# Zilong-Li/BaseVarC

Measured on AMD Instinct MI355X. Metric: sites/sec at N=1e6 samples; achieved HBM GB/s vs roofline, higher is better.
Workload: dtype f64

## Files before the change

basevarc_amd/csrc/bgzf_deflate_kernel.hip:

```cpp
#include "bvc_device.h"
#include "bvc_internal.h"
#include "crc32_device.h"

namespace bvc {

namespace {

constexpr int kBdThreads = 1024;
constexpr int kBdRound = 256;
constexpr int kBdLanes = kBdThreads / kBdRound;
constexpr int kBdWays = 16, kBdHashBits = 11, kBdHash = 1 << kBdHashBits;
constexpr int kBdWaysPerLane = kBdWays / kBdLanes;
constexpr uint32_t kBdIn = BVC_BGZF_BLOCK_INPUT;
constexpr uint32_t kBdSlot = 65536;
constexpr uint32_t kBdMinMatch = 4, kBdMaxMatch = 258, kBdMaxDist = 32768;
constexpr uint32_t kBdMatchBit = 0x80000000u;
constexpr int kBdInWords = kBdSlot / 4 + 4;
constexpr int kBdTabWords = kBdWays / 2 * kBdHash;
constexpr int kBdBitWords = kBdHash;
static_assert(kBdTabWords * 4 >= (int)kBdIn && kBdBitWords * 32 >= (int)kBdIn && kBdHash == 2048, "what takes the tables' place fits");
static_assert((kBdInWords + kBdTabWords + 2 * kBdBitWords + 32) * 4 <= 160 * 1024, "one workgroup's LDS");
static_assert(kBdIn % 64 == 0 && kBdIn / 64 <= kBdThreads, "64 positions a thread in pass C");
static_assert(kBdWays == 16 && kBdRound == 256, "the packing of the table's and the round's cells");

struct BlockDesc { int64_t src; uint32_t len; uint32_t pad; };

__device__ __forceinline__ uint32_t ld32(const uint32_t *w, uint32_t a)
{
    const uint32_t i = a >> 2;
    const uint64_t v = (uint64_t)w[i] | ((uint64_t)w[i + 1] << 32);
    return (uint32_t)(v >> ((a & 3u) * 8u));
}

__device__ __forceinline__ uint32_t hash_of(uint32_t four) { return (four * 2654435761u) >> (32 - kBdHashBits); }

__device__ __forceinline__ uint32_t rev_bits(uint32_t x, uint32_t n) { return __brev(x) >> (32u - n); }

__device__ __forceinline__ uint32_t literal_bits(uint32_t b, uint32_t &bits)
{
    if (b < 144u) { bits = rev_bits(0x30u + b, 8u); return 8u; }
    bits = rev_bits(0x190u + (b - 144u), 9u);
    return 9u;
}
__device__ __forceinline__ uint32_t match_bits(uint32_t len, uint32_t dist, uint32_t &bits)
{
    const uint32_t l = len - 3u;
    uint32_t sym, le = 0u, lx = 0u;
    if (len == 258u) sym = 285u;
    else if (l < 8u) sym = 257u + l;
    else { le = (31u - (uint32_t)__clz((int)l)) - 2u; sym = 261u + 4u * le + ((l >> le) & 3u); lx = l & ((1u << le) - 1u); }
    uint32_t n;
    if (sym <= 279u) { bits = rev_bits(sym - 256u, 7u); n = 7u; } else { bits = rev_bits(0xC0u + (sym - 280u), 8u); n = 8u; }
    bits |= lx << n; n += le;
    const uint32_t d = dist - 1u;
    uint32_t ds, de = 0u, dx = 0u;
    if (d < 4u) ds = d;
    else { de = (31u - (uint32_t)__clz((int)d)) - 1u; ds = 2u * de + 2u + ((d >> de) & 1u); dx = d & ((1u << de) - 1u); }
    bits |= rev_bits(ds, 5u) << n; n += 5u;
    bits |= dx << n; n += de;
    return n;
}

}

__global__ __launch_bounds__(256) void bgzf_plan_kernel(
    int64_t n_pieces, const int64_t *__restrict__ piece_off, const int64_t *__restrict__ piece_len, const int64_t *__restrict__ first_block,
    int64_t n_blocks, BlockDesc *__restrict__ desc)
{
    for (int64_t b = (int64_t)blockIdx.x * 256 + threadIdx.x; b < n_blocks; b += (int64_t)gridDim.x * 256) {
        int64_t lo = 0, hi = n_pieces - 1;
        while (lo < hi) {
            const int64_t mid = (lo + hi + 1) >> 1;
            if (first_block[mid] <= b) lo = mid; else hi = mid - 1;
        }
        const int64_t at = (b - first_block[lo]) * (int64_t)kBdIn, left = piece_len[lo] - at;
        BlockDesc d;
        d.src = piece_off[lo] + at;
        d.len = left <= 0 ? 0u : (left < (int64_t)kBdIn ? (uint32_t)left : kBdIn);
        d.pad = 0u;
        desc[b] = d;
    }
}

__global__ __launch_bounds__(kBdThreads) void bgzf_deflate_kernel(
    const uint8_t *__restrict__ data, const BlockDesc *__restrict__ desc, int64_t n_blocks, uint8_t *__restrict__ staging,
    uint32_t *__restrict__ bsize, uint32_t *__restrict__ match_rows)
{
    BVC_POISON_LDS();
    __shared__ __attribute__((aligned(16))) uint32_t s_in[kBdInWords];
    __shared__ __attribute__((aligned(16))) uint32_t s_tab[kBdTabWords];
    __shared__ uint32_t s_first[kBdBitWords];
    __shared__ uint32_t s_path[kBdBitWords];
    __shared__ uint32_t s_scan[32];
    const uint32_t tid = threadIdx.x, lane = tid & (kWave - 1), wave = tid >> 6;
    uint32_t *const match = match_rows + (size_t)blockIdx.x * kBdIn;
    uint32_t *const s_out = s_in;
    uint8_t *const s_sym = reinterpret_cast<uint8_t *>(s_tab);
    uint32_t *const s_ism = s_first;

    for (int64_t blk = blockIdx.x; blk < n_blocks; blk += gridDim.x) {
        const uint32_t n = desc[blk].len < kBdIn ? desc[blk].len : kBdIn;
        uint8_t *const slot = staging + (size_t)blk * kBdSlot;
        if (n == 0u) {
            if (tid == 0u) bsize[blk] = 0u;
            continue;
        }
        const uint8_t *__restrict__ src = data + desc[blk].src;
        {
            const uint32_t head = (uint32_t)(reinterpret_cast<uintptr_t>(src) & 3u);
            const uint32_t *__restrict__ g = reinterpret_cast<const uint32_t *>(src - head);
            for (uint32_t w = tid; w < (uint32_t)kBdInWords; w += kBdThreads) {
                uint32_t v = 0u;
                if (4u * w < n) {
                    const uint32_t lo = g[w];
                    const uint32_t hi = head != 0u && 4u * (w + 1u) < n + head ? g[w + 1u] : 0u;
                    v = (uint32_t)((((uint64_t)hi << 32) | lo) >> (8u * head));
                    const uint32_t left = n - 4u * w;
                    if (left < 4u) v &= (1u << (8u * left)) - 1u;
                }
                s_in[w] = v;
            }
        }
        for (uint32_t w = tid; w < (uint32_t)kBdTabWords; w += kBdThreads) s_tab[w] = 0u;
        for (uint32_t w = tid; w < (uint32_t)kBdBitWords; w += kBdThreads) s_first[w] = 0u;
        __syncthreads();

        const uint32_t sub = tid & (kBdLanes - 1), slotpos = tid / kBdLanes;
        const uint32_t rounds = (n + kBdRound - 1) / kBdRound;
        uint32_t prev_h = 0u, prev_p = 0u;
        bool prev_ok = false;
        for (uint32_t r = 0; r < rounds; ++r) {
            const uint32_t p = r * kBdRound + slotpos;
            const bool ok = p + 4u <= n;
            const uint32_t four = ok ? ld32(s_in, p) : 0u;
            const uint32_t h = hash_of(four);
            if (sub == 0u) {
                if (prev_ok && BVC_LDS_OK(0x901, prev_h, kBdHash)) {
                    const uint32_t way = (r - 1u) & (kBdWays - 1u);
                    uint32_t *const cell = &s_tab[(way & 7u) * kBdHash + prev_h];
                    const uint32_t cur = *cell;
                    atomicMax(cell, way >> 3 ? (cur & 0xFFFFu) | ((prev_p + 1u) << 16) : (cur & 0xFFFF0000u) | (prev_p + 1u));
                }
                if (ok && BVC_LDS_OK(0x902, h, kBdHash)) atomicMax(&s_first[h], ((r + 1u) << 8) | (255u - slotpos));
            }
            __syncthreads();
            uint32_t best = 0u, best_d = 0u;
            if (ok) {
                const uint32_t mx = n - p < kBdMaxMatch ? n - p : kBdMaxMatch;
                auto consider = [&](uint32_t q) {
                    const uint32_t d = p - q;
                    if (d > kBdMaxDist || best == mx) return;
                    if (best >= kBdMinMatch && ld32(s_in, q + best - 3u) != ld32(s_in, p + best - 3u)) return;
                    uint32_t l = 0u;
                    while (l < mx) {
                        const uint32_t x = ld32(s_in, q + l) ^ ld32(s_in, p + l);
                        if (x != 0u) { l += (uint32_t)__builtin_ctz(x) >> 3; break; }
                        l += 4u;
                    }
                    l = l < mx ? l : mx;
                    if (l > best) { best = l; best_d = d; }
                };
#pragma unroll
                for (uint32_t k = 0; k < (uint32_t)kBdWaysPerLane; ++k) {
                    const uint32_t way = sub * kBdWaysPerLane + k;
                    const uint32_t cell = s_tab[(way & 7u) * kBdHash + h];
                    const uint32_t q1 = way >> 3 ? cell >> 16 : cell & 0xFFFFu;
                    if (q1 != 0u && q1 - 1u < p && BVC_LDS_OK(0x903, q1 - 1u, kBdIn)) consider(q1 - 1u);
                }
                if (sub == 0u) {
                    const uint32_t f = s_first[h];
                    const uint32_t q = r * kBdRound + 255u - (f & 255u);
                    if ((f >> 8) == r + 1u && q < p && BVC_LDS_OK(0x904, q, kBdIn)) consider(q);
                }
            }
            uint32_t key = best >= kBdMinMatch ? (best << 16) | (kBdMaxDist - best_d) : 0u;
#pragma unroll
            for (int d = 1; d < kBdLanes; d <<= 1) {
                const uint32_t o = (uint32_t)__shfl_xor((int)key, d);
                key = o > key ? o : key;
            }
            if (sub == 0u && p < n)
                match[p] = key != 0u ? kBdMatchBit | (((key >> 16) - 3u) << 16) | (kBdMaxDist - (key & 0xFFFFu) - 1u) : 0u;
            prev_h = h; prev_p = p; prev_ok = ok;
            __syncthreads();
        }
        __threadfence();
        __syncthreads();

        for (uint32_t g = tid; g < kBdIn / 32u; g += kBdThreads) {
            uint32_t ism = 0u;
#pragma unroll
            for (uint32_t j = 0; j < 8u; ++j) {
                const uint32_t p0 = 32u * g + 4u * j;
                uint32_t packed = 0u;
                if (p0 < n) {
                    const uint4 m4 = *reinterpret_cast<const uint4 *>(match + p0);
                    const uint32_t m[4] = {m4.x, m4.y, m4.z, m4.w};
                    const uint32_t lit = s_in[p0 >> 2];
#pragma unroll
                    for (uint32_t k = 0; k < 4u; ++k) {
                        const bool is = p0 + k < n && (m[k] & kBdMatchBit) != 0u;
                        ism |= is ? 1u << (4u * j + k) : 0u;
                        packed |= (is ? (m[k] >> 16) & 0xFFu : (lit >> (8u * k)) & 0xFFu) << (8u * k);
                    }
                }
                s_tab[8u * g + j] = packed;
            }
            s_ism[g] = ism;
            s_path[g] = 0u;
        }
        __syncthreads();
        if (tid == 0u) {
            uint32_t p = 0u;
            while (p < n) {
                const uint32_t w = p >> 5, b = p & 31u;
                const uint32_t m = s_ism[w] >> b;
                if (m == 0u) { s_path[w] |= ~0u << b; p = (w + 1u) << 5; continue; }
                const uint32_t k = (uint32_t)__builtin_ctz(m);
                s_path[w] |= (((1u << k) - 1u) | (1u << k)) << b;
                p += k;
                p += (uint32_t)s_sym[p] + 3u;
            }
        }
        __syncthreads();

        uint32_t my_bits = 0u;
        uint64_t mask = 0u;
        const uint32_t base = 64u * tid;
        if (base < n) {
            mask = (uint64_t)s_path[2u * tid] | ((uint64_t)s_path[2u * tid + 1u] << 32);
            if (n - base < 64u) mask &= (1ull << (n - base)) - 1ull;
            const uint64_t ism = (uint64_t)s_ism[2u * tid] | ((uint64_t)s_ism[2u * tid + 1u] << 32);
            for (uint64_t left = mask; left != 0u; left &= left - 1u) {
                const uint32_t p = base + (uint32_t)__builtin_ctzll(left);
                uint32_t bits;
                my_bits += (ism >> (p - base)) & 1u ? match_bits((uint32_t)s_sym[p] + 3u, (match[p] & 0x7FFFu) + 1u, bits)
                                                   : literal_bits(s_sym[p], bits);
            }
        }
        uint32_t incl = my_bits;
#pragma unroll
        for (int d = 1; d < kWave; d <<= 1) {
            const uint32_t o = (uint32_t)__shfl_up((int)incl, d);
            incl += lane >= (uint32_t)d ? o : 0u;
        }
        if (lane == kWave - 1) s_scan[wave] = incl;
        __syncthreads();
        uint32_t before = 0u, all = 0u;
#pragma unroll
        for (uint32_t v = 0; v < kBdThreads / kWave; ++v) {
            const uint32_t s = s_scan[v];
            before += v < wave ? s : 0u;
            all += s;
        }
        const uint32_t total_bits = 3u + all + 7u;
        const uint32_t coded = (total_bits + 7u) >> 3;
        const bool stored = coded > n + 5u;
        const uint32_t csize = stored ? n + 5u : coded;
        const uint32_t out_words = (csize + 3u) >> 2;
        if (!stored) {
            for (uint32_t w = tid; w < out_words; w += kBdThreads) s_out[w] = 0u;
            __syncthreads();
            if (base < n) {
                uint32_t at = 3u + before + incl - my_bits;
                uint32_t word = at >> 5, fill = at & 31u;
                uint64_t acc = tid == 0u ? 3u : 0u;
                const uint64_t ism = (uint64_t)s_ism[2u * tid] | ((uint64_t)s_ism[2u * tid + 1u] << 32);
                for (uint64_t left = mask; left != 0u; left &= left - 1u) {
                    const uint32_t p = base + (uint32_t)__builtin_ctzll(left);
                    uint32_t bits;
                    const uint32_t nb = (ism >> (p - base)) & 1u ? match_bits((uint32_t)s_sym[p] + 3u, (match[p] & 0x7FFFu) + 1u, bits)
                                                                : literal_bits(s_sym[p], bits);
                    acc |= (uint64_t)bits << fill;
                    fill += nb;
                    if (fill >= 32u) {
                        if (BVC_LDS_OK(0x905, word, out_words)) atomicOr(&s_out[word], (uint32_t)acc);
                        acc >>= 32; fill -= 32u; ++word;
                    }
                }
                if (acc != 0u && BVC_LDS_OK(0x906, word, out_words)) atomicOr(&s_out[word], (uint32_t)acc);
            }
            __syncthreads();
        }
        const uint32_t bs = csize + 26u;
        {
            auto byte_at = [&](uint32_t x) -> uint32_t {
                if (x < 18u) {
                    const uint32_t word = x < 4u ? 0x04088b1fu : x < 8u ? 0u : x < 12u ? 0x0006ff00u : x < 16u ? 0x00024342u : (bs - 1u) & 0xFFFFu;
                    return (word >> (8u * (x & 3u))) & 0xFFu;
                }
                const uint32_t i = x - 18u;
                if (i < csize) {
                    if (!stored) return (s_out[i >> 2] >> (8u * (i & 3u))) & 0xFFu;
                    if (i < 5u) return ((i < 4u ? 0x01u | (n << 8) | ((~n & 0xFFu) << 24) : (~n >> 8) & 0xFFu) >> (8u * (i & 3u))) & 0xFFu;
                    return (s_in[(i - 5u) >> 2] >> (8u * ((i - 5u) & 3u))) & 0xFFu;
                }
                const uint32_t t = i - csize;
                return t >= 4u && t < 8u ? (n >> (8u * (t - 4u))) & 0xFFu : 0u;
            };
            uint32_t *const slot32 = reinterpret_cast<uint32_t *>(slot);
            const uint32_t first = stored ? 23u : 18u;
            for (uint32_t k = tid; 4u * k < bs; k += kBdThreads) {
                uint32_t v;
                if (4u * k >= first && 4u * k + 4u <= 18u + csize) v = ld32(stored ? s_in : s_out, 4u * k - first);
                else v = byte_at(4u * k) | (byte_at(4u * k + 1u) << 8) | (byte_at(4u * k + 2u) << 16) | (byte_at(4u * k + 3u) << 24);
                slot32[k] = v;
            }
        }
        if (tid == 0u) bsize[blk] = bs;
        __syncthreads();
    }
}

__global__ __launch_bounds__(kWave) void bgzf_crc_kernel(const uint8_t *__restrict__ data16, uint32_t shift, const BlockDesc *__restrict__ desc,
                                                         int64_t n_blocks, const uint32_t *__restrict__ bsize, uint8_t *__restrict__ staging)
{
    BVC_POISON_LDS();
    __shared__ uint32_t tab[256];
    const int lane = threadIdx.x;
    crc_table_fill(tab, lane);
    for (int64_t blk = blockIdx.x; blk < n_blocks; blk += gridDim.x) {
        const uint32_t n = desc[blk].len < kBdIn ? desc[blk].len : kBdIn;
        if (n == 0u) continue;
        const uint32_t crc = crc32_wave(data16, (uint64_t)desc[blk].src + shift, n, tab, lane);
        const uint32_t bs = bsize[blk] <= kBdSlot ? bsize[blk] : kBdSlot;
        if (lane < 4 && bs >= 26u) staging[(size_t)blk * kBdSlot + bs - 8u + (uint32_t)lane] = (uint8_t)(crc >> (8 * lane));
    }
}

__global__ __launch_bounds__(1024) void bgzf_scan_kernel(int64_t n_blocks, const uint32_t *__restrict__ bsize, int64_t *__restrict__ block_off,
                                                         int64_t n_pieces, const int64_t *__restrict__ first_block, int64_t *__restrict__ comp_off)
{
    BVC_POISON_LDS();
    __shared__ int64_t s_sz[1024];
    const int tid = threadIdx.x;
    int64_t base = 0;
    for (int64_t b0 = 0; b0 < n_blocks; b0 += 1024) {
        const int64_t b = b0 + tid;
        const int64_t sz = b < n_blocks ? (int64_t)bsize[b] : 0;
        s_sz[tid] = sz;
        __syncthreads();
        for (int d = 1; d < 1024; d <<= 1) {
            const int64_t v = tid >= d ? s_sz[tid - d] : 0;
            __syncthreads();
            s_sz[tid] += v;
            __syncthreads();
        }
        if (b < n_blocks) block_off[b] = base + s_sz[tid] - sz;
        const int64_t tot = s_sz[1023];
        __syncthreads();
        base += tot;
    }
    if (tid == 0) block_off[n_blocks] = base;
    __threadfence();
    __syncthreads();
    for (int64_t i = tid; i <= n_pieces; i += 1024) comp_off[i] = block_off[first_block[i]];
}

__global__ __launch_bounds__(256) void bgzf_pack_kernel(int64_t n_blocks, const uint32_t *__restrict__ bsize, const int64_t *__restrict__ block_off,
                                                        const uint8_t *__restrict__ staging, uint8_t *__restrict__ comp, int64_t comp_cap)
{
    if (block_off[n_blocks] > comp_cap) return;
    for (int64_t blk = blockIdx.x; blk < n_blocks; blk += gridDim.x) {
        const uint32_t bs = bsize[blk] <= kBdSlot - 8u ? bsize[blk] : kBdSlot - 8u;
        const uint32_t *__restrict__ from = reinterpret_cast<const uint32_t *>(staging + (size_t)blk * kBdSlot);
        uint8_t *__restrict__ to = comp + block_off[blk];
        const uint32_t lead = (uint32_t)(-reinterpret_cast<uintptr_t>(to) & 3u);
        const uint32_t head = lead < bs ? lead : bs, words = (bs - head) >> 2, tail = head + 4u * words;
        if (threadIdx.x < head) to[threadIdx.x] = (uint8_t)(from[0] >> (8u * threadIdx.x));
        uint32_t *__restrict__ to32 = reinterpret_cast<uint32_t *>(to + head);
        for (uint32_t j = threadIdx.x; j < words; j += 256) {
            const uint32_t at = head + 4u * j;
            const uint64_t v = (uint64_t)from[at >> 2] | ((uint64_t)from[(at >> 2) + 1u] << 32);
            to32[j] = (uint32_t)(v >> (8u * (at & 3u)));
        }
        if (threadIdx.x < bs - tail) {
            const uint32_t at = tail + threadIdx.x;
            to[at] = (uint8_t)(from[at >> 2] >> (8u * (at & 3u)));
        }
    }
}

size_t bgzf_deflate_scratch_bytes(int64_t n_pieces, int64_t n_blocks)
{
    Layout L;
    (void)bgzf_deflate_scratch(nullptr, n_pieces, n_blocks, &L);
    return L.at;
}

BgzfDeflateScratch bgzf_deflate_scratch(void *buf, int64_t n_pieces, int64_t n_blocks, Layout *sized)
{
    Layout L{reinterpret_cast<uintptr_t>(buf)};
    const size_t nb = (size_t)n_blocks, grid = nb < (size_t)kBgzfDeflateGrid ? nb : (size_t)kBgzfDeflateGrid;
    BgzfDeflateScratch s;
    s.first_block = L.take<int64_t>((size_t)n_pieces + 1);
    s.block_off = L.take<int64_t>(nb + 1);
    s.desc = L.take<char>(nb * sizeof(BlockDesc));
    s.bsize = L.take<uint32_t>(nb);
    s.match_rows = L.take<uint32_t>(grid * kBdIn);
    s.staging = L.take<uint8_t>(nb * kBdSlot);
    if (sized) *sized = L;
    return s;
}

hipError_t launch_bgzf_deflate(hipStream_t stream, int64_t n_pieces, const uint8_t *data, const int64_t *piece_off, const int64_t *piece_len,
                               int64_t n_blocks, const BgzfDeflateScratch &s, uint8_t *comp, int64_t comp_cap, int64_t *comp_off)
{
    BlockDesc *const desc = reinterpret_cast<BlockDesc *>(s.desc);
    if (n_blocks > 0) {
        const unsigned grid = (unsigned)(n_blocks < kBgzfDeflateGrid ? n_blocks : kBgzfDeflateGrid);
        hipLaunchKernelGGL(bgzf_plan_kernel, dim3((unsigned)((n_blocks + 255) / 256 < 1024 ? (n_blocks + 255) / 256 : 1024)), dim3(256), 0, stream,
                           n_pieces, piece_off, piece_len, s.first_block, n_blocks, desc);
        hipLaunchKernelGGL(bgzf_deflate_kernel, dim3(grid), dim3(kBdThreads), 0, stream, data, desc, n_blocks, s.staging, s.bsize, s.match_rows);
        const uintptr_t a = reinterpret_cast<uintptr_t>(data);
        hipLaunchKernelGGL(bgzf_crc_kernel, dim3((unsigned)(n_blocks < 65536 ? n_blocks : 65536)), dim3(kWave), 0, stream,
                           reinterpret_cast<const uint8_t *>(a & ~(uintptr_t)15), (uint32_t)(a & 15u), desc, n_blocks, s.bsize, s.staging);
    }
    hipLaunchKernelGGL(bgzf_scan_kernel, dim3(1), dim3(1024), 0, stream, n_blocks, s.bsize, s.block_off, n_pieces, s.first_block, comp_off);
    if (n_blocks > 0)
        hipLaunchKernelGGL(bgzf_pack_kernel, dim3((unsigned)(n_blocks < 2048 ? n_blocks : 2048)), dim3(256), 0, stream, n_blocks, s.bsize,
                           s.block_off, s.staging, comp, comp_cap);
    return hipGetLastError();
}

#ifdef BVC_CHECK_LDS
BVC_DEFINE_DEBUG_READER(debug_read_bgzf_deflate)
#endif

}
```

Measured before the change: 3.377 million.

## Parallelize deflate match search within quads and chunk the greedy parse path

Match finding now screens all candidates with a 16-byte compare, then extends surviving candidates cooperatively across the four lanes of a quad using DPP min/max reductions and 8-byte loads, instead of each lane walking its candidates serially. The match-row store is deferred past the next barrier. The single-thread greedy parse over the whole block becomes a per-64-position chunk exit table computed in parallel, so one thread only hops between chunks and each thread then rebuilds its own path mask. ld32 uses alignbyte, and the stored-block fallback reloads the input. This aims to cut divergent serial match loops and the serial parse, at the cost of more code complexity and extra LDS traffic.

New measurement: 3.375 million (median of 2 runs). Within noise of the previous version (-0.1%).

```diff
diff --git a/basevarc_amd/csrc/bgzf_deflate_kernel.hip b/basevarc_amd/csrc/bgzf_deflate_kernel.hip
--- a/basevarc_amd/csrc/bgzf_deflate_kernel.hip
+++ b/basevarc_amd/csrc/bgzf_deflate_kernel.hip
@@ -15,21 +15,89 @@
 constexpr uint32_t kBdSlot = 65536;
 constexpr uint32_t kBdMinMatch = 4, kBdMaxMatch = 258, kBdMaxDist = 32768;
 constexpr uint32_t kBdMatchBit = 0x80000000u;
+constexpr uint32_t kBdScreen = 16;
+constexpr uint32_t kBdChunk = 64;
+constexpr uint32_t kBdNone = 0xFFFFFFFFu;
 constexpr int kBdInWords = kBdSlot / 4 + 4;
 constexpr int kBdTabWords = kBdWays / 2 * kBdHash;
 constexpr int kBdBitWords = kBdHash;
 static_assert(kBdTabWords * 4 >= (int)kBdIn && kBdBitWords * 32 >= (int)kBdIn && kBdHash == 2048, "what takes the tables' place fits");
 static_assert((kBdInWords + kBdTabWords + 2 * kBdBitWords + 32) * 4 <= 160 * 1024, "one workgroup's LDS");
-static_assert(kBdIn % 64 == 0 && kBdIn / 64 <= kBdThreads, "64 positions a thread in pass C");
+static_assert(kBdChunk == 64 && kBdIn % kBdChunk == 0 && kBdIn / kBdChunk <= kBdThreads, "64 positions a thread in passes B and C: one 64-bit mask");
+static_assert(kBdLanes == 4 && kBdWaysPerLane == 4 && kBdScreen == 16, "a quad a position in pass A, four words screened");
+static_assert(kBdChunk - 1 + kBdMaxMatch - kBdChunk < 512, "a chunk's exit, relative to its end, in nine bits");
 static_assert(kBdWays == 16 && kBdRound == 256, "the packing of the table's and the round's cells");
 
 struct BlockDesc { int64_t src; uint32_t len; uint32_t pad; };
 
+#ifdef BVC_DIAG_KNOBS
+#define BVC_BD_STOP_PARAM , int dbg_stop
+#define BVC_BD_STOP_ARG , bgzf_dbg_stop()
+#define BVC_BD_STOP(k)                                                                                            \
+    if (dbg_stop == (k)) {                                                                                        \
+        if (tid == 0u) bsize[blk] = 0u;                                                                           \
+        __syncthreads();                                                                                          \
+        continue;                                                                                                 \
+    }
+#else
+#define BVC_BD_STOP_PARAM
+#define BVC_BD_STOP_ARG
+#define BVC_BD_STOP(k)
+#endif
+
 __device__ __forceinline__ uint32_t ld32(const uint32_t *w, uint32_t a)
 {
     const uint32_t i = a >> 2;
-    const uint64_t v = (uint64_t)w[i] | ((uint64_t)w[i + 1] << 32);
-    return (uint32_t)(v >> ((a & 3u) * 8u));
+    return __builtin_amdgcn_alignbyte(w[i + 1], w[i], a & 3u);
+}
+__device__ __forceinline__ uint64_t ld64_aligned(const uint32_t *w, uint32_t a)
+{
+    const uint32_t i = a >> 2;
+    return (uint64_t)w[i] | ((uint64_t)w[i + 1] << 32);
+}
+__device__ __forceinline__ uint64_t ld64(const uint32_t *w, uint32_t a)
+{
+    const uint32_t i = a >> 2, by = a & 3u;
+    const uint32_t w0 = w[i], w1 = w[i + 1], w2 = w[i + 2];
+    return (uint64_t)__builtin_amdgcn_alignbyte(w1, w0, by) | ((uint64_t)__builtin_amdgcn_alignbyte(w2, w1, by) << 32);
+}
+__device__ __forceinline__ void ld128(const uint32_t *w, uint32_t a, uint32_t (&b)[4])
+{
+    const uint32_t i = a >> 2, by = a & 3u;
+    const uint32_t w0 = w[i], w1 = w[i + 1], w2 = w[i + 2], w3 = w[i + 3], w4 = w[i + 4];
+    b[0] = __builtin_amdgcn_alignbyte(w1, w0, by);
+    b[1] = __builtin_amdgcn_alignbyte(w2, w1, by);
+    b[2] = __builtin_amdgcn_alignbyte(w3, w2, by);
+    b[3] = __builtin_amdgcn_alignbyte(w4, w3, by);
+}
+__device__ __forceinline__ uint32_t first_difference(uint32_t x0, uint32_t x1, uint32_t x2, uint32_t x3)
+{
+    const uint32_t lo = x0 != 0u ? x0 : x1, hi = x2 != 0u ? x2 : x3;
+    const uint32_t at_lo = x0 != 0u ? 0u : 4u, at_hi = x2 != 0u ? 8u : 12u;
+    const bool in_lo = (x0 | x1) != 0u;
+    const uint32_t x = in_lo ? lo : hi, at = in_lo ? at_lo : at_hi;
+    return x != 0u ? at + ((uint32_t)__builtin_ctz(x) >> 3) : 16u;
+}
+
+template <int XOR>
+__device__ __forceinline__ uint32_t quad_xor(uint32_t v)
+{
+    static_assert(XOR == 1 || XOR == 2, "inside a quad");
+    return (uint32_t)__builtin_amdgcn_update_dpp(0, (int)v, XOR == 1 ? 0xB1 : 0x4E, 0xF, 0xF, false);
+}
+__device__ __forceinline__ uint32_t quad_max(uint32_t v)
+{
+    const uint32_t a = quad_xor<1>(v);
+    v = a > v ? a : v;
+    const uint32_t b = quad_xor<2>(v);
+    return b > v ? b : v;
+}
+__device__ __forceinline__ uint32_t quad_min(uint32_t v)
+{
+    const uint32_t a = quad_xor<1>(v);
+    v = a < v ? a : v;
+    const uint32_t b = quad_xor<2>(v);
+    return b < v ? b : v;
 }
 
 __device__ __forceinline__ uint32_t hash_of(uint32_t four) { return (four * 2654435761u) >> (32 - kBdHashBits); }
@@ -84,7 +152,7 @@
 
 __global__ __launch_bounds__(kBdThreads) void bgzf_deflate_kernel(
     const uint8_t *__restrict__ data, const BlockDesc *__restrict__ desc, int64_t n_blocks, uint8_t *__restrict__ staging,
-    uint32_t *__restrict__ bsize, uint32_t *__restrict__ match_rows)
+    uint32_t *__restrict__ bsize, uint32_t *__restrict__ match_rows BVC_BD_STOP_PARAM)
 {
     BVC_POISON_LDS();
     __shared__ __attribute__((aligned(16))) uint32_t s_in[kBdInWords];
@@ -96,6 +164,7 @@
     uint32_t *const match = match_rows + (size_t)blockIdx.x * kBdIn;
     uint32_t *const s_out = s_in;
     uint8_t *const s_sym = reinterpret_cast<uint8_t *>(s_tab);
+    uint8_t *const s_exit = reinterpret_cast<uint8_t *>(s_in);
     uint32_t *const s_ism = s_first;
 
     for (int64_t blk = blockIdx.x; blk < n_blocks; blk += gridDim.x) {
@@ -106,7 +175,7 @@
             continue;
         }
         const uint8_t *__restrict__ src = data + desc[blk].src;
-        {
+        auto load_input = [&]() {
             const uint32_t head = (uint32_t)(reinterpret_cast<uintptr_t>(src) & 3u);
             const uint32_t *__restrict__ g = reinterpret_cast<const uint32_t *>(src - head);
             for (uint32_t w = tid; w < (uint32_t)kBdInWords; w += kBdThreads) {
@@ -120,20 +189,23 @@
                 }
                 s_in[w] = v;
             }
-        }
+        };
+        load_input();
         for (uint32_t w = tid; w < (uint32_t)kBdTabWords; w += kBdThreads) s_tab[w] = 0u;
         for (uint32_t w = tid; w < (uint32_t)kBdBitWords; w += kBdThreads) s_first[w] = 0u;
         __syncthreads();
+        BVC_BD_STOP(1)
 
         const uint32_t sub = tid & (kBdLanes - 1), slotpos = tid / kBdLanes;
         const uint32_t rounds = (n + kBdRound - 1) / kBdRound;
-        uint32_t prev_h = 0u, prev_p = 0u;
-        bool prev_ok = false;
+        uint32_t prev_h = 0u, prev_p = 0u, prev_m = 0u;
+        bool prev_ok = false, prev_store = false;
         for (uint32_t r = 0; r < rounds; ++r) {
             const uint32_t p = r * kBdRound + slotpos;
             const bool ok = p + 4u <= n;
-            const uint32_t four = ok ? ld32(s_in, p) : 0u;
-            const uint32_t h = hash_of(four);
+            uint32_t at_p[4] = {0u, 0u, 0u, 0u};
+            if (ok) ld128(s_in, p, at_p);
+            const uint32_t h = hash_of(at_p[0]);
             if (sub == 0u) {
                 if (prev_ok && BVC_LDS_OK(0x901, prev_h, kBdHash)) {
                     const uint32_t way = (r - 1u) & (kBdWays - 1u);
@@ -144,48 +216,75 @@
                 if (ok && BVC_LDS_OK(0x902, h, kBdHash)) atomicMax(&s_first[h], ((r + 1u) << 8) | (255u - slotpos));
             }
             __syncthreads();
-            uint32_t best = 0u, best_d = 0u;
+            if (prev_store) match[prev_p] = prev_m;
+            uint32_t key = 0u;
             if (ok) {
                 const uint32_t mx = n - p < kBdMaxMatch ? n - p : kBdMaxMatch;
-                auto consider = [&](uint32_t q) {
-                    const uint32_t d = p - q;
-                    if (d > kBdMaxDist || best == mx) return;
-                    if (best >= kBdMinMatch && ld32(s_in, q + best - 3u) != ld32(s_in, p + best - 3u)) return;
-                    uint32_t l = 0u;
-                    while (l < mx) {
-                        const uint32_t x = ld32(s_in, q + l) ^ ld32(s_in, p + l);
-                        if (x != 0u) { l += (uint32_t)__builtin_ctz(x) >> 3; break; }
-                        l += 4u;
-                    }
-                    l = l < mx ? l : mx;
-                    if (l > best) { best = l; best_d = d; }
-                };
+                uint32_t cand[kBdWaysPerLane + 1];
+                bool has[kBdWaysPerLane + 1];
 #pragma unroll
                 for (uint32_t k = 0; k < (uint32_t)kBdWaysPerLane; ++k) {
                     const uint32_t way = sub * kBdWaysPerLane + k;
                     const uint32_t cell = s_tab[(way & 7u) * kBdHash + h];
                     const uint32_t q1 = way >> 3 ? cell >> 16 : cell & 0xFFFFu;
-                    if (q1 != 0u && q1 - 1u < p && BVC_LDS_OK(0x903, q1 - 1u, kBdIn)) consider(q1 - 1u);
-                }
-                if (sub == 0u) {
+                    has[k] = q1 != 0u && q1 - 1u < p && p - (q1 - 1u) <= kBdMaxDist && BVC_LDS_OK(0x903, q1 - 1u, kBdIn);
+                    cand[k] = has[k] ? q1 - 1u : p;
+                }
+                {
                     const uint32_t f = s_first[h];
                     const uint32_t q = r * kBdRound + 255u - (f & 255u);
-                    if ((f >> 8) == r + 1u && q < p && BVC_LDS_OK(0x904, q, kBdIn)) consider(q);
-                }
-            }
-            uint32_t key = best >= kBdMinMatch ? (best << 16) | (kBdMaxDist - best_d) : 0u;
-#pragma unroll
-            for (int d = 1; d < kBdLanes; d <<= 1) {
-                const uint32_t o = (uint32_t)__shfl_xor((int)key, d);
-                key = o > key ? o : key;
-            }
-            if (sub == 0u && p < n)
-                match[p] = key != 0u ? kBdMatchBit | (((key >> 16) - 3u) << 16) | (kBdMaxDist - (key & 0xFFFFu) - 1u) : 0u;
+                    has[kBdWaysPerLane] = sub == 0u && (f >> 8) == r + 1u && q < p && BVC_LDS_OK(0x904, q, kBdIn);
+                    cand[kBdWaysPerLane] = has[kBdWaysPerLane] ? q : p;
+                }
+                uint32_t surv[kBdWaysPerLane + 1];
+#pragma unroll
+                for (uint32_t k = 0; k <= (uint32_t)kBdWaysPerLane; ++k) {
+                    uint32_t at_q[4];
+                    ld128(s_in, cand[k], at_q);
+                    uint32_t m = first_difference(at_q[0] ^ at_p[0], at_q[1] ^ at_p[1], at_q[2] ^ at_p[2], at_q[3] ^ at_p[3]);
+                    m = m < mx ? m : mx;
+                    const bool more = m == kBdScreen && mx > kBdScreen;
+                    surv[k] = has[k] && more ? cand[k] + 1u : 0u;
+                    const uint32_t mk = has[k] && !more && m >= kBdMinMatch ? (m << 16) | (kBdMaxDist - (p - cand[k])) : 0u;
+                    key = mk > key ? mk : key;
+                }
+                uint32_t best = 0u, best_d = 0u;
+                for (;;) {
+                    uint32_t mine = surv[0];
+#pragma unroll
+                    for (uint32_t k = 1; k <= (uint32_t)kBdWaysPerLane; ++k) mine = surv[k] > mine ? surv[k] : mine;
+                    const uint32_t top = quad_max(mine);
+                    if (top == 0u || best == mx) break;
+#pragma unroll
+                    for (uint32_t k = 0; k <= (uint32_t)kBdWaysPerLane; ++k) surv[k] = surv[k] == top ? 0u : surv[k];
+                    const uint32_t q = top - 1u;
+                    if (best != 0u && ld32(s_in, q + best - 3u) != ld32(s_in, p + best - 3u)) continue;
+                    const uint32_t o0 = kBdScreen - (p & 3u);
+                    uint32_t l = mx;
+                    for (uint32_t o = o0; o < mx; o += 8u * kBdLanes) {
+                        const uint32_t mo = o + 8u * sub;
+                        uint32_t miss = kBdNone;
+                        if (mo < mx) {
+                            const uint64_t x = ld64(s_in, q + mo) ^ ld64_aligned(s_in, p + mo);
+                            if (x != 0u) miss = mo + ((uint32_t)__builtin_ctzll(x) >> 3);
+                        }
+                        miss = quad_min(miss);
+                        if (miss != kBdNone) { l = miss < mx ? miss : mx; break; }
+                    }
+                    if (l > best) { best = l; best_d = p - q; }
+                }
+                if (best != 0u) key = (best << 16) | (kBdMaxDist - best_d);
+                key = quad_max(key);
+            }
+            prev_store = sub == 0u && p < n;
+            prev_m = key != 0u ? kBdMatchBit | (((key >> 16) - 3u) << 16) | (kBdMaxDist - (key & 0xFFFFu) - 1u) : 0u;
             prev_h = h; prev_p = p; prev_ok = ok;
             __syncthreads();
         }
+        if (prev_store) match[prev_p] = prev_m;
         __threadfence();
         __syncthreads();
+        BVC_BD_STOP(2)
 
         for (uint32_t g = tid; g < kBdIn / 32u; g += kBdThreads) {
             uint32_t ism = 0u;
@@ -207,30 +306,57 @@
                 s_tab[8u * g + j] = packed;
             }
             s_ism[g] = ism;
-            s_path[g] = 0u;
+        }
+        __syncthreads();
+        const uint32_t base = kBdChunk * tid;
+        uint64_t ism = 0u, mask = 0u;
+        if (base < n) {
+            ism = (uint64_t)s_ism[2u * tid] | ((uint64_t)s_ism[2u * tid + 1u] << 32);
+            uint64_t ninth = 0u;
+            uint32_t leave = 0u;
+            for (int i = (int)kBdChunk - 1; i >= 0; --i) {
+                if ((ism >> i) & 1u) {
+                    const uint32_t to = (uint32_t)i + (uint32_t)s_sym[base + (uint32_t)i] + 3u;
+                    leave = to >= kBdChunk ? to - kBdChunk
+                                          : (uint32_t)s_exit[base + to] | ((uint32_t)(ninth >> to) & 1u) << 8;
+                }
+                s_exit[base + (uint32_t)i] = (uint8_t)leave;
+                ninth |= (uint64_t)(leave >> 8) << i;
+            }
+            s_path[2u * tid] = (uint32_t)ninth;
+            s_path[2u * tid + 1u] = (uint32_t)(ninth >> 32);
         }
         __syncthreads();
         if (tid == 0u) {
             uint32_t p = 0u;
-            while (p < n) {
-                const uint32_t w = p >> 5, b = p & 31u;
-                const uint32_t m = s_ism[w] >> b;
-                if (m == 0u) { s_path[w] |= ~0u << b; p = (w + 1u) << 5; continue; }
-                const uint32_t k = (uint32_t)__builtin_ctz(m);
-                s_path[w] |= (((1u << k) - 1u) | (1u << k)) << b;
-                p += k;
-                p += (uint32_t)s_sym[p] + 3u;
-            }
-        }
-        __syncthreads();
+            for (uint32_t c = 0; kBdChunk * c < n; ++c) {
+                uint32_t enters = kBdNone;
+                const uint32_t end = kBdChunk * (c + 1u);
+                if (p < end && p < n && BVC_LDS_OK(0x907, p, kBdIn)) {
+                    enters = p - kBdChunk * c;
+                    const uint32_t nine = (s_path[2u * c + (enters >> 5)] >> (enters & 31u)) & 1u;
+                    p = end + (uint32_t)s_exit[p] + (nine << 8);
+                }
+                s_path[2u * c] = enters;
+            }
+        }
+        __syncthreads();
+        if (base < n) {
+            uint32_t at = s_path[2u * tid];
+            while (at < kBdChunk) {
+                const uint64_t m = ism >> at;
+                if (m == 0u) { mask |= ~0ull << at; break; }
+                const uint32_t k = (uint32_t)__builtin_ctzll(m);
+                mask |= ((2ull << k) - 1ull) << at;
+                at += k;
+                at += (uint32_t)s_sym[base + at] + 3u;
+            }
+            if (n - base < kBdChunk) mask &= (1ull << (n - base)) - 1ull;
+        }
+        BVC_BD_STOP(3)
 
         uint32_t my_bits = 0u;
-        uint64_t mask = 0u;
-        const uint32_t base = 64u * tid;
         if (base < n) {
-            mask = (uint64_t)s_path[2u * tid] | ((uint64_t)s_path[2u * tid + 1u] << 32);
-            if (n - base < 64u) mask &= (1ull << (n - base)) - 1ull;
-            const uint64_t ism = (uint64_t)s_ism[2u * tid] | ((uint64_t)s_ism[2u * tid + 1u] << 32);
             for (uint64_t left = mask; left != 0u; left &= left - 1u) {
                 const uint32_t p = base + (uint32_t)__builtin_ctzll(left);
                 uint32_t bits;
@@ -265,7 +391,6 @@
                 uint32_t at = 3u + before + incl - my_bits;
                 uint32_t word = at >> 5, fill = at & 31u;
                 uint64_t acc = tid == 0u ? 3u : 0u;
-                const uint64_t ism = (uint64_t)s_ism[2u * tid] | ((uint64_t)s_ism[2u * tid + 1u] << 32);
                 for (uint64_t left = mask; left != 0u; left &= left - 1u) {
                     const uint32_t p = base + (uint32_t)__builtin_ctzll(left);
                     uint32_t bits;
@@ -280,6 +405,9 @@
                 }
                 if (acc != 0u && BVC_LDS_OK(0x906, word, out_words)) atomicOr(&s_out[word], (uint32_t)acc);
             }
+            __syncthreads();
+        } else {
+            load_input();
             __syncthreads();
         }
         const uint32_t bs = csize + 26u;
@@ -403,6 +531,15 @@
     return s;
 }
 
+#ifdef BVC_DIAG_KNOBS
+static int bgzf_dbg_stop()
+{
+    const char *e = getenv("BVC_DBG_DEFLATE_STOP");
+    const int v = e ? atoi(e) : 0;
+    return v >= 1 && v <= 3 ? v : 0;
+}
+#endif
+
 hipError_t launch_bgzf_deflate(hipStream_t stream, int64_t n_pieces, const uint8_t *data, const int64_t *piece_off, const int64_t *piece_len,
                                int64_t n_blocks, const BgzfDeflateScratch &s, uint8_t *comp, int64_t comp_cap, int64_t *comp_off)
 {
@@ -411,7 +548,7 @@
         const unsigned grid = (unsigned)(n_blocks < kBgzfDeflateGrid ? n_blocks : kBgzfDeflateGrid);
         hipLaunchKernelGGL(bgzf_plan_kernel, dim3((unsigned)((n_blocks + 255) / 256 < 1024 ? (n_blocks + 255) / 256 : 1024)), dim3(256), 0, stream,
                            n_pieces, piece_off, piece_len, s.first_block, n_blocks, desc);
-        hipLaunchKernelGGL(bgzf_deflate_kernel, dim3(grid), dim3(kBdThreads), 0, stream, data, desc, n_blocks, s.staging, s.bsize, s.match_rows);
+        hipLaunchKernelGGL(bgzf_deflate_kernel, dim3(grid), dim3(kBdThreads), 0, stream, data, desc, n_blocks, s.staging, s.bsize, s.match_rows BVC_BD_STOP_ARG);
         const uintptr_t a = reinterpret_cast<uintptr_t>(data);
         hipLaunchKernelGGL(bgzf_crc_kernel, dim3((unsigned)(n_blocks < 65536 ? n_blocks : 65536)), dim3(kWave), 0, stream,
                            reinterpret_cast<const uint8_t *>(a & ~(uintptr_t)15), (uint32_t)(a & 15u), desc, n_blocks, s.bsize, s.staging);
```
